# bentherien/point-cloud-reid

Hardware: AMD Instinct MI355X
Metric: siamese pair-comparisons/sec @1024 pts (higher is better)
Workload: dtype bf16x3

## Files before the change

point-cloud-reid_amd/csrc/attn_kernels_impl.h:

```cpp
#pragma once
#ifndef PCR_ATTN_PREC
#define PCR_ATTN_PREC 0
#endif
#include "tile_dense.h"

#include <stdio.h>

#include <vector>

namespace {
constexpr int kAPrec = PCR_ATTN_PREC;
struct AttnArgs {
  pcr_attn_params p;
  int dbg;
  int wpc;
};

constexpr int kATraceWgs = 512, kATraceRecs = 24, kATraceMarks = 8;
__device__ unsigned long long g_attn_trace[2 * kATraceWgs * kATraceRecs * kATraceMarks];


__device__ __forceinline__ void pos_hidden(float *dst, int RP, const float *P, const float *w0,
                                           const float *b0, int d, int T) {
  for (int e = threadIdx.x; e < d * T; e += blockDim.x) {
// ... 1346 lines not shown
          }
        }
    }
    __builtin_amdgcn_wave_barrier();
    PCR_AMARK(7);
    PCR_ANEXT();
  }
#undef PCR_AMARK
#undef PCR_ANEXT
}

template <int NB, bool TRANS = false>
__device__ __forceinline__ void ap128_step(f32x16 (&acc)[NB], const bf16x8 *wb, int ls, const bf16x8 &bh, const bf16x8 &bl) {
  auto mm = [](const bf16x8 &w, const bf16x8 &x, const f32x16 &c) __attribute__((always_inline)) {
    return TRANS ? __builtin_amdgcn_mfma_f32_32x32x16_bf16(x, w, c, 0, 0, 0) : __builtin_amdgcn_mfma_f32_32x32x16_bf16(w, x, c, 0, 0, 0);
  };
#pragma unroll
  for (int c0 = 0; c0 < NB; c0 += 4) {
    bf16x8 wh[4], wl[4];
#pragma unroll
    for (int cb = 0; cb < 4; cb++) {
      wh[cb] = wb[((ls * NB + c0 + cb) * 2) * 64];
      wl[cb] = wb[((ls * NB + c0 + cb) * 2 + 1) * 64];
    }
#pragma unroll
    for (int cb = 0; cb < 4; cb++) acc[c0 + cb] = mm(wh[cb], bh, acc[c0 + cb]);
#pragma unroll
    for (int cb = 0; cb < 4; cb++) acc[c0 + cb] = mm(wh[cb], bl, acc[c0 + cb]);
#pragma unroll
    for (int cb = 0; cb < 4; cb++) acc[c0 + cb] = mm(wl[cb], bh, acc[c0 + cb]);
    asm volatile("" ::: "memory");
  }
}
constexpr int kAp128Waves = 4, kAp128ChunkU = 2048, kAp128Chunks = 16;
constexpr int kAp128Npc = kAp128ChunkU / (64 * kAp128Waves);
__device__ __forceinline__ void ring128_fetch(f32x4 (&stg)[kAp128Npc], __amdgpu_buffer_rsrc_t r, int kk, int tid) {
#pragma unroll
  for (int u = 0; u < kAp128Npc; u++)
    stg[u] = __builtin_bit_cast(f32x4, __builtin_amdgcn_raw_buffer_load_b128(r, tid * 16, (kk * kAp128ChunkU + u * 64 * kAp128Waves) * 16, 0));
  asm volatile("" ::: "memory");
}
__device__ __forceinline__ void ring128_commit(f32x4 *s_ring, const f32x4 (&stg)[kAp128Npc], int k, int tid) {
  f32x4 *dst = s_ring + (k & 1) * kAp128ChunkU + tid;
#pragma unroll
  for (int u = 0; u < kAp128Npc; u++) dst[u * 64 * kAp128Waves] = stg[u];
  __syncthreads();
}
constexpr size_t kAp128Lds = (size_t)2 * kAp128ChunkU * 16 + (640 + 4 * 128 + kAp128Waves * 128) * sizeof(float);
template <int NH>
__global__ __launch_bounds__(64 * kAp128Waves) __attribute__((amdgpu_waves_per_eu(1, 1)))
void attn_apply_stream128_kernel(AttnArgs a) {
  constexpr int D = 128, ND = 4, SD = 8, GPH = 8 / NH;
  extern __shared__ __attribute__((aligned(16))) float smem[];
  const pcr_attn_params &p = a.p;
  f32x4 *s_ring = reinterpret_cast<f32x4 *>(smem);
  int coff = 2 * kAp128ChunkU * 4;
  asm volatile("" : "+s"(coff));
  float *s_c = smem + coff;
  f32x4 *s_p0 = reinterpret_cast<f32x4 *>(s_c + 640);
  float *s_ks = s_c + 640 + 4 * 128;
  const int tid = threadIdx.x, lane = tid & 63, j = lane & 31, h = lane >> 5;
  const int wave = __builtin_amdgcn_readfirstlane(tid >> 6);
  const __amdgpu_buffer_rsrc_t rwq = __builtin_amdgcn_make_buffer_rsrc(const_cast<float *>(p.wq), 0, 4 * kAp128ChunkU * 16, 0x00020000),
                               rw0 = __builtin_amdgcn_make_buffer_rsrc(const_cast<float *>(p.wmlp0), 0, 8 * kAp128ChunkU * 16, 0x00020000),
                               rw2 = __builtin_amdgcn_make_buffer_rsrc(const_cast<float *>(p.wmlp2), 0, 4 * kAp128ChunkU * 16, 0x00020000);
  f32x4 stg[kAp128Npc];
  auto fetch = [&](int k) __attribute__((always_inline)) {
    k %= kAp128Chunks;
    ring128_fetch(stg, k < 4 ? rwq : (k < 12 ? rw0 : rw2), k < 4 ? k : (k < 12 ? k - 4 : k - 12), tid);
  };
  auto commit = [&](int k) __attribute__((always_inline)) { ring128_commit(s_ring, stg, k, tid); };
  for (int e = tid; e < D; e += 64 * kAp128Waves) {
    s_c[e] = p.bq[e];
    s_c[128 + e] = p.ln1_g[e];
    s_c[256 + e] = p.ln1_b[e];
    s_c[384 + e] = p.ln2_g[e];
    s_c[512 + e] = p.ln2_b[e];
    s_p0[e] = f32x4{p.pos0_w[3 * e], p.pos0_w[3 * e + 1], p.pos0_w[3 * e + 2], p.pos0_b[e]};
  }
  fetch(0);
  commit(0);
  const int nblk = p.Lq >> 5;
  const long nitem = (long)p.B * nblk;
  const float skf = (float)p.Sk;
  float *ksw = s_ks + wave * 128;
  auto cvec = [&](const float *base, int cb, int g) __attribute__((always_inline)) {
    return *reinterpret_cast<const f32x4 *>(base + 32 * cb + 8 * g + 4 * h);
  };
  auto to_ops = [&](const f32x16 &acc, int G, bf16x8 &oh, bf16x8 &ol) __attribute__((always_inline)) {
    float v[8];
#pragma unroll
    for (int e = 0; e < 8; e++) v[e] = acc[8 * G + e];
    bf_split8(v, oh, ol, true);
  };
  auto layernorm = [&](f32x16 (&v)[ND], const float *gam, const float *bet) __attribute__((always_inline)) {
    float sm = 0.f;
#pragma unroll
    for (int cb = 0; cb < ND; cb++)
#pragma unroll
      for (int r = 0; r < 16; r++) sm += v[cb][r];
    sm += __shfl_xor(sm, 32, 64);
    const float mean = sm / (float)D;
    float vr = 0.f;
#pragma unroll
    for (int cb = 0; cb < ND; cb++)
#pragma unroll
      for (int r = 0; r < 16; r++) {
        const float dlt = v[cb][r] - mean;
        vr += dlt * dlt;
      }
    vr += __shfl_xor(vr, 32, 64);
    const float inv = 1.0f / sqrtf(vr / (float)D + 1e-5f);
#pragma unroll
    for (int cb = 0; cb < ND; cb++)
#pragma unroll
      for (int g = 0; g < 4; g++) {
        const f32x4 gv = cvec(gam, cb, g), bv = cvec(bet, cb, g);
#pragma unroll
        for (int qq = 0; qq < 4; qq++) v[cb][4 * g + qq] = (v[cb][4 * g + qq] - mean) * inv * gv[qq] + bv[qq];
      }
  };
  for (long it0 = (long)blockIdx.x * kAp128Waves; it0 < nitem; it0 += (long)gridDim.x * kAp128Waves) {
    const long item = it0 + wave;
    const bool live = item < nitem;
    const long it = live ? item : nitem - 1;
    const long b = it / nblk;
    const int blk = (int)(it - b * nblk);
    const size_t bq_ = p.q_index ? (size_t)p.q_index[b] : (size_t)b;
    const size_t kb_ = p.kv_index ? (size_t)p.kv_index[b] : (size_t)b;
    const float *kvp = p.kv + kb_ * ((size_t)D * D + D);
    const int t = blk * 32 + j;
    const __amdgpu_buffer_rsrc_t rfeat = __builtin_amdgcn_make_buffer_rsrc(
        const_cast<float *>(p.feat_q + bq_ * D * p.Lq), 0, D * p.Lq * 4, 0x00020000);
    const int vo = (4 * h * p.Lq + t) * 4;
    auto load_x = [&](float (&xf)[64]) __attribute__((always_inline)) {
#pragma unroll
      for (int e = 0; e < 64; e++) {
        const int ch = 16 * (e >> 3) + bf_kpos(0, e & 7);
        xf[e] = __builtin_bit_cast(float, __builtin_amdgcn_raw_buffer_load_b32(rfeat, vo, ch * p.Lq * 4, 0));
      }
    };
    ksw[lane] = kvp[(size_t)D * D + lane];
    ksw[64 + lane] = kvp[(size_t)D * D + 64 + lane];
    bf16x8 bh[16], bl[16];
    {
      float xf[64];
      load_x(xf);
      const float *xyz = p.xyz_q + (bq_ * p.Lq + t) * 3;
      const float px = xyz[0], py = xyz[1], pz = xyz[2];
#pragma unroll
      for (int s2 = 0; s2 < SD; s2++) {
        float hv[8];
#pragma unroll
        for (int e = 0; e < 8; e++) {
          const f32x4 w = s_p0[16 * s2 + bf_kpos(0, e) + 4 * h];
          const float v = w[0] * px + w[1] * py + w[2] * pz + w[3];
          hv[e] = relu_i(v);
        }
        bf_split8(hv, bh[SD + s2], bl[SD + s2], true);
      }
#pragma unroll
      for (int e = 0; e < 64; e++) asm volatile("" : "+v"(xf[e]));
#pragma unroll
      for (int s2 = 0; s2 < SD; s2++) {
        float xv[8];
#pragma unroll
        for (int e = 0; e < 8; e++) xv[e] = xf[8 * s2 + e];
        bf_split8(xv, bh[s2], bl[s2], true);
      }
    }
    f32x16 q[ND];
#pragma unroll
    for (int cb = 0; cb < ND; cb++)
#pragma unroll
      for (int g = 0; g < 4; g++) {
        const f32x4 bqv = cvec(s_c, cb, g);
#pragma unroll
        for (int qq = 0; qq < 4; qq++) q[cb][4 * g + qq] = bqv[qq];
      }
#pragma unroll
    for (int k = 0; k < 4; k++) {
      fetch(k + 1);
      const bf16x8 *wb = reinterpret_cast<const bf16x8 *>(s_ring + (k & 1) * kAp128ChunkU) + lane;
#pragma unroll
      for (int ls = 0; ls < 4; ls++) ap128_step<ND>(q, wb, ls, bh[4 * k + ls], bl[4 * k + ls]);
      commit(k + 1);
    }
    float zg[SD];
#pragma unroll
    for (int cb = 0; cb < ND; cb++)
#pragma unroll
      for (int g = 0; g < 4; g++) {
        const f32x4 ksv = cvec(ksw, cb, g);
        float zz = 0.f;
#pragma unroll
        for (int qq = 0; qq < 4; qq++) {
          const float v = elu1(q[cb][4 * g + qq]);
          q[cb][4 * g + qq] = v;
          zz += v * ksv[qq];
        }
        if ((g & 1) == 0) zg[2 * cb + (g >> 1)] = zz;
        else zg[2 * cb + (g >> 1)] += zz;
      }
    float zs[NH];
#pragma unroll
    for (int hd = 0; hd < NH; hd++) {
      float z = zg[hd * GPH];
#pragma unroll
      for (int gi = 1; gi < GPH; gi++) z += zg[hd * GPH + gi];
      z += __shfl_xor(z, 32, 64);
      zs[hd] = (1.0f / (z + 1e-6f)) * skf;
    }
#pragma unroll
    for (int cb = 0; cb < ND; cb++)
#pragma unroll
      for (int r = 0; r < 16; r++) q[cb][r] *= zs[(2 * cb + (r >> 3)) / GPH];
    {
      bf16x8 ch_[SD], cl_[SD];
#pragma unroll
      for (int cb = 0; cb < ND; cb++)
#pragma unroll
        for (int G = 0; G < 2; G++) to_ops(q[cb], G, ch_[2 * cb + G], cl_[2 * cb + G]);
#pragma unroll
      for (int cb = 0; cb < ND; cb++)
#pragma unroll
        for (int r = 0; r < 16; r++) q[cb][r] = 0.f;
      const bf16x8 *mb = reinterpret_cast<const bf16x8 *>(kvp) + lane;
      bf16x8 mh[2][ND], ml[2][ND];
#pragma unroll
      for (int cb = 0; cb < ND; cb++) {
        mh[0][cb] = mb[(cb * 2) * 64];
        ml[0][cb] = mb[(cb * 2 + 1) * 64];
      }
#pragma unroll
      for (int s2 = 0; s2 < SD; s2++) {
        const int c = s2 & 1;
        if (s2 + 1 < SD) {
#pragma unroll
          for (int cb = 0; cb < ND; cb++) {
            mh[c ^ 1][cb] = mb[(((s2 + 1) * ND + cb) * 2) * 64];
            ml[c ^ 1][cb] = mb[(((s2 + 1) * ND + cb) * 2 + 1) * 64];
          }
        }
        asm volatile("" ::: "memory");
#pragma unroll
        for (int cb = 0; cb < ND; cb++) q[cb] = __builtin_amdgcn_mfma_f32_32x32x16_bf16(mh[c][cb], ch_[s2], q[cb], 0, 0, 0);
#pragma unroll
        for (int cb = 0; cb < ND; cb++) q[cb] = __builtin_amdgcn_mfma_f32_32x32x16_bf16(mh[c][cb], cl_[s2], q[cb], 0, 0, 0);
#pragma unroll
        for (int cb = 0; cb < ND; cb++) q[cb] = __builtin_amdgcn_mfma_f32_32x32x16_bf16(ml[c][cb], ch_[s2], q[cb], 0, 0, 0);
      }
    }
    layernorm(q, s_c + 128, s_c + 256);
#pragma unroll
    for (int cb = 0; cb < ND; cb++)
#pragma unroll
      for (int G = 0; G < 2; G++) to_ops(q[cb], G, bh[SD + 2 * cb + G], bl[SD + 2 * cb + G]);
    f32x16 f[2 * ND];
#pragma unroll
    for (int cb = 0; cb < 2 * ND; cb++)
#pragma unroll
      for (int r = 0; r < 16; r++) f[cb][r] = 0.f;
#pragma unroll
    for (int k = 4; k < 12; k++) {
      fetch(k + 1);
      const bf16x8 *wb = reinterpret_cast<const bf16x8 *>(s_ring + (k & 1) * kAp128ChunkU) + lane;
#pragma unroll
      for (int ls = 0; ls < 2; ls++) ap128_step<2 * ND>(f, wb, ls, bh[2 * (k - 4) + ls], bl[2 * (k - 4) + ls]);
      commit(k + 1);
    }
    float xf[64];
    load_x(xf);
    f32x16 o[ND];
#pragma unroll
    for (int cb = 0; cb < ND; cb++)
#pragma unroll
      for (int r = 0; r < 16; r++) o[cb][r] = 0.f;
#pragma unroll
    for (int k = 12; k < 16; k++) {
      fetch(k + 1);
      bf16x8 oh[4], ol[4];
#pragma unroll
      for (int i = 0; i < 2; i++) {
        f32x16 &fc = f[2 * (k - 12) + i];
#pragma unroll
        for (int r = 0; r < 16; r++) fc[r] = relu_i(fc[r]);
#pragma unroll
        for (int G = 0; G < 2; G++) to_ops(fc, G, oh[2 * i + G], ol[2 * i + G]);
      }
      const bf16x8 *wb = reinterpret_cast<const bf16x8 *>(s_ring + (k & 1) * kAp128ChunkU) + lane;
#pragma unroll
      for (int ls = 0; ls < 4; ls++) ap128_step<ND>(o, wb, ls, oh[ls], ol[ls]);
      commit(k + 1);
    }
    layernorm(o, s_c + 384, s_c + 512);
#pragma unroll
    for (int cb = 0; cb < ND; cb++)
#pragma unroll
      for (int r = 0; r < 16; r++) o[cb][r] += xf[16 * cb + r];
    if (live) {
      const __amdgpu_buffer_rsrc_t rout =
          __builtin_amdgcn_make_buffer_rsrc(p.out + (size_t)b * D * p.Lq, 0, D * p.Lq * 4, 0x00020000);
#pragma unroll
      for (int e = 0; e < 16 * ND; e++) {
        const int ch = 16 * (e >> 3) + bf_kpos(0, e & 7);
        const float v = o[e >> 4][e & 15];
        __builtin_amdgcn_raw_buffer_store_b32(__builtin_bit_cast(unsigned, v), rout, vo, ch * p.Lq * 4, 0);
      }
    }
  }
}

__host__ __device__ constexpr int attn_kv128_wpc(int nblk) { return nblk >= 32 ? 4 : (nblk >= 16 ? 2 : 1); }
constexpr size_t kKv128Lds0 = (size_t)2 * kAp128ChunkU * 16 + 128 * 16 + 256 * 4;
template <int NH>
__global__ __launch_bounds__(64 * kAp128Waves) __attribute__((amdgpu_waves_per_eu(1, 1)))
void attn_kv_stream128_kernel(AttnArgs a) {
  constexpr int D = 128, SD = 8, TPH = 4 / NH, NKV = NH * TPH * TPH;
  constexpr int KVU = NKV * 16 + 4;
  typedef unsigned u32x4 __attribute__((ext_vector_type(4)));
  extern __shared__ __attribute__((aligned(16))) float smem[];
  const pcr_attn_params &p = a.p;
  f32x4 *s_ring = reinterpret_cast<f32x4 *>(smem);
  int coff = 2 * kAp128ChunkU * 4;
  asm volatile("" : "+s"(coff));
  f32x4 *s_p0 = reinterpret_cast<f32x4 *>(smem + coff);
  float *s_bkv = smem + coff + 4 * D;
  float *s_red = s_bkv + 2 * D;
  const int tid = threadIdx.x, lane = tid & 63, j = lane & 31, h = lane >> 5;
  const int wave = __builtin_amdgcn_readfirstlane(tid >> 6);
  const __amdgpu_buffer_rsrc_t rw = __builtin_amdgcn_make_buffer_rsrc(const_cast<float *>(p.wkv_bf), 0, 8 * kAp128ChunkU * 16, 0x00020000);
  f32x4 stg[kAp128Npc];
  auto fetch = [&](int k) __attribute__((always_inline)) { ring128_fetch(stg, rw, k & 7, tid); };
  auto commit = [&](int k) __attribute__((always_inline)) { ring128_commit(s_ring, stg, k, tid); };
  for (int e = tid; e < D; e += 64 * kAp128Waves) s_p0[e] = f32x4{p.pos0_w[3 * e], p.pos0_w[3 * e + 1], p.pos0_w[3 * e + 2], p.pos0_b[e]};
  for (int e = tid; e < 2 * D; e += 64 * kAp128Waves) s_bkv[e] = p.bkv[e];
  fetch(0);
  commit(0);
  const int Sk = p.Sk, nblk = Sk >> 5;
  const int wpc = a.wpc, cpg = kAp128Waves / wpc;
  const int cslot = wave / wpc, wsub = wave - cslot * wpc;
  const int nper = (nblk + wpc - 1) / wpc;
  const long cstep = (long)gridDim.x * cpg;
  const float inv_sk = 1.0f / (float)Sk;
  float xf[64], pxyz[3];
  auto issue = [&](long bq, int blk) __attribute__((always_inline)) {
    const __amdgpu_buffer_rsrc_t rfeat =
        __builtin_amdgcn_make_buffer_rsrc(const_cast<float *>(p.feat_k + (size_t)bq * D * Sk), 0, D * Sk * 4, 0x00020000);
    const int t = blk * 32 + j, vo = (4 * h * Sk + t) * 4;
#pragma unroll
    for (int e = 0; e < 64; e++) {
      const int ch = 16 * (e >> 3) + bf_kpos(0, e & 7);
      xf[e] = __builtin_bit_cast(float, __builtin_amdgcn_raw_buffer_load_b32(rfeat, vo, ch * Sk * 4, 0));
    }
    const __amdgpu_buffer_rsrc_t rxyz =
        __builtin_amdgcn_make_buffer_rsrc(const_cast<float *>(p.xyz_k + (size_t)bq * Sk * 3), 0, Sk * 12, 0x00020000);
#pragma unroll
    for (int c = 0; c < 3; c++) pxyz[c] = __builtin_bit_cast(float, __builtin_amdgcn_raw_buffer_load_b32(rxyz, t * 12, c * 4, 0));
    asm volatile("" ::: "memory");
  };
  if ((long)blockIdx.x * cpg + cslot < p.B && wsub < nblk) issue((long)blockIdx.x * cpg + cslot, wsub);
  for (long c0 = (long)blockIdx.x * cpg; c0 < p.B; c0 += cstep) {
    const long b = c0 + cslot;
    const bool live = b < p.B;
    f32x16 kv[NKV];
#pragma unroll
    for (int i = 0; i < NKV; i++)
#pragma unroll
      for (int r = 0; r < 16; r++) kv[i][r] = 0.f;
    float ks[4] = {0.f, 0.f, 0.f, 0.f};
    for (int it = 0; it < nper; it++) {
      const int blk = wsub + it * wpc;
      const bool has = live && blk < nblk;
      const bool last = it + 1 == nper;
      const long bn = last ? b + cstep : b;
      const int blkn = last ? wsub : blk + wpc;
      const bool hasn = bn < p.B && blkn < nblk;
      bf16x8 bh[SD], bl[SD];
      if (has) {
#pragma unroll
        for (int s2 = 0; s2 < SD; s2++) {
          float xv[8];
#pragma unroll
          for (int e = 0; e < 8; e++) xv[e] = xf[8 * s2 + e];
          bf_split8(xv, bh[s2], bl[s2], true);
        }
      }
      f32x16 acc[8];
#pragma unroll
      for (int cb = 0; cb < 8; cb++)
#pragma unroll
        for (int r = 0; r < 16; r++) acc[cb][r] = 0.f;
#pragma unroll
      for (int k = 0; k < 8; k++) {
        fetch(k + 1);
        if (has) {
          const bf16x8 *wb = reinterpret_cast<const bf16x8 *>(s_ring + (k & 1) * kAp128ChunkU) + lane;
#pragma unroll
          for (int ls = 0; ls < 2; ls++) {
            if (k < 4) {
              ap128_step<8, true>(acc, wb, ls, bh[2 * k + ls], bl[2 * k + ls]);
            } else {
              const int s2 = 2 * k + ls - SD;
              float hv[8];
#pragma unroll
              for (int e = 0; e < 8; e++) {
                const f32x4 w = s_p0[16 * s2 + bf_kpos(0, e) + 4 * h];
                const float v = w[0] * pxyz[0] + w[1] * pxyz[1] + w[2] * pxyz[2] + w[3];
                hv[e] = relu_i(v);
              }
              bf16x8 hh, hl;
              bf_split8(hv, hh, hl, true);
              ap128_step<8, true>(acc, wb, ls, hh, hl);
            }
          }
        }
        commit(k + 1);
      }
      if (hasn) issue(bn, blkn);
      else {
#pragma unroll
        for (int e = 0; e < 64; e++) xf[e] = 0.f;
        pxyz[0] = pxyz[1] = pxyz[2] = 0.f;
      }
      if (has) {
        float bias[8];
#pragma unroll
        for (int cb = 0; cb < 8; cb++) bias[cb] = s_bkv[cb * 32 + j];
#pragma unroll
        for (int r = 0; r < 16; r++) {
#pragma unroll
          for (int cb = 0; cb < 4; cb++) {
            acc[cb][r] = elu1(acc[cb][r] + bias[cb]);
            ks[cb] += acc[cb][r];
            acc[4 + cb][r] = (acc[4 + cb][r] + bias[4 + cb]) * inv_sk;
          }
        }
#pragma unroll
        for (int i = 0; i < NKV; i++) {
          const int hd = i / (TPH * TPH), ib = hd * TPH + (i % (TPH * TPH)) / TPH, jb = hd * TPH + i % TPH;
#pragma unroll
          for (int r = 0; r < 16; r++) kv[i] = __builtin_amdgcn_mfma_f32_32x32x2f32(acc[4 + jb][r], acc[ib][r], kv[i], 0, 0, 0);
        }
      }
    }
#pragma unroll
    for (int cb = 0; cb < 4; cb++) ks[cb] += __shfl_xor(ks[cb], 32, 64);
    if (wpc > 1) {
      int ln = lane;
      asm volatile("" : "+v"(ln));
      float *red = s_red + (size_t)cslot * KVU * 64 + ln;
      for (int round = 0; round < wpc; round++) {
        if (wsub == round) {
#pragma unroll
          for (int i = 0; i < NKV; i++)
#pragma unroll
            for (int r = 0; r < 16; r++) {
              float *dst = red + (i * 16 + r) * 64;
              *dst = round == 0 ? kv[i][r] : *dst + kv[i][r];
            }
#pragma unroll
          for (int cb = 0; cb < 4; cb++) {
            float *dst = red + (NKV * 16 + cb) * 64;
            *dst = round == 0 ? ks[cb] : *dst + ks[cb];
          }
        }
        __syncthreads();
      }
#pragma unroll
      for (int i = 0; i < NKV; i++)
#pragma unroll
        for (int r = 0; r < 16; r++) kv[i][r] = red[(i * 16 + r) * 64];
#pragma unroll
      for (int cb = 0; cb < 4; cb++) ks[cb] = red[(NKV * 16 + cb) * 64];
    }
    if (live) {
      int ln = lane;
      asm volatile("" : "+v"(ln));
      const int j = ln & 31, h = ln >> 5;
      const __amdgpu_buffer_rsrc_t rkv =
          __builtin_amdgcn_make_buffer_rsrc(p.kv + (size_t)b * ((size_t)D * D + D), 0, (D * D + D) * 4, 0x00020000);
      const __amdgpu_buffer_rsrc_t rwm = __builtin_amdgcn_make_buffer_rsrc(const_cast<float *>(p.wmerge), 0, D * D * 4, 0x00020000);
      for (int ob = wsub; ob < 4; ob += wpc) {
        const int wrow = ((ob * 32 + j) * D + 4 * h) * 4;
#pragma unroll
        for (int hd = 0; hd < NH; hd++) {
          f32x4 w[TPH][4];
#pragma unroll
          for (int jj = 0; jj < TPH; jj++)
#pragma unroll
            for (int g = 0; g < 4; g++)
              w[jj][g] = __builtin_bit_cast(f32x4, __builtin_amdgcn_raw_buffer_load_b128(rwm, wrow, ((hd * TPH + jj) * 32 + 8 * g) * 4, 0));
#pragma unroll
          for (int dl = 0; dl < TPH; dl++) {
            const int db = hd * TPH + dl;
            f32x16 m;
#pragma unroll
            for (int r = 0; r < 16; r++) m[r] = 0.f;
#pragma unroll
            for (int jj = 0; jj < TPH; jj++) {
              const int i = hd * TPH * TPH + dl * TPH + jj;
#pragma unroll
              for (int r = 0; r < 16; r++) m = __builtin_amdgcn_mfma_f32_32x32x2f32(kv[i][r], w[jj][r >> 2][r & 3], m, 0, 0, 0);
            }
#pragma unroll
            for (int G = 0; G < 2; G++) {
              float v[8];
#pragma unroll
              for (int e = 0; e < 8; e++) v[e] = m[8 * G + e];
              bf16x8 hi, lo;
              bf_split8(v, hi, lo, true);
              const int unit = (((db * 2 + G) * (D >> 5) + ob) * 2) * 64 + h * 32 + j;
              __builtin_amdgcn_raw_buffer_store_b128(__builtin_bit_cast(u32x4, hi), rkv, unit * 16, 0, 0);
              __builtin_amdgcn_raw_buffer_store_b128(__builtin_bit_cast(u32x4, lo), rkv, (unit + 64) * 16, 0, 0);
            }
          }
        }
      }
      if (wsub == 0 && h == 0) {
#pragma unroll
        for (int cb = 0; cb < 4; cb++)
          __builtin_amdgcn_raw_buffer_store_b32(__builtin_bit_cast(unsigned, ks[cb]), rkv, (D * D + cb * 32 + j) * 4, 0, 0);
      }
    }
  }
}
#endif

}

static int attn_check(const pcr_attn_params &p) {
  if (p.B < 0 || p.Lq < 1 || p.Sk < 1 || p.c1 < 1 || p.c2 < 1 || p.cout < 1 || p.nhead < 1) return 1;
  if (p.d < 32 || p.d > 512 || (p.d & 31) || p.d % p.nhead) return 1;
  if (p.d > 128 && ((p.d & 63) || ((p.d / p.nhead) & 63) || p.d / p.nhead > 256)) return 1;
  if ((p.c2 & 7) || p.cout > 512 || p.cfinal > 512) return 1;
  if (!p.feat_q || !p.feat_k || !p.xyz_k || !p.kv || !p.pos0_w || !p.pos0_b || !p.wq || !p.bq || !p.wkv ||
      !p.bkv || !p.wmerge || !p.wmlp0 || !p.wmlp2 || !p.ln1_g || !p.ln1_b || !p.ln2_g || !p.ln2_b)
    return 1;
  if (p.q_pos && (!p.xyz_q || p.c1 != p.c2 || p.c1 != p.d)) return 1;
  if (p.residual && p.cout != p.c1) return 1;
  if (p.cfinal && (!p.wfinal || !p.bfinal || (p.cout & 7))) return 1;
  return 0;
}

static void attn_dump_trace(const char *path, const char *tag, int wgs, int B, int Sk) {
  static int launches = 0;
  static const int skip = pcr_tune_int("PCR_SA_TRACE_SKIP");
  launches++;
  if (launches <= skip || launches > skip + 8) return;
  static std::vector<unsigned long long> host(2 * kATraceWgs * kATraceRecs * kATraceMarks);
  if (hipDeviceSynchronize() != hipSuccess) return;
  if (hipMemcpyFromSymbol(host.data(), HIP_SYMBOL(g_attn_trace), host.size() * sizeof(unsigned long long)) != hipSuccess) return;
  FILE *f = fopen(path, "a");
  if (!f) return;
  const int n = 2 * (wgs < kATraceWgs ? wgs : kATraceWgs);
  fprintf(f, "launch %d kernel %s wgs %d B %d Sk %d\n", launches, tag, wgs, B, Sk);
  for (int w = 0; w < n; w++) {
    const unsigned long long *t = host.data() + (size_t)w * (kATraceRecs * kATraceMarks);
// ... 60 lines not shown
    if (onew)
      rc = mh ? pcr_launch_lds<attn_kv_stream64_kernel<true, kBfUnit, 4, kBfUnit>>(gg, bb, lds_s, st, a)
              : pcr_launch_lds<attn_kv_stream64_kernel<false, kBfUnit, 4, kBfUnit>>(gg, bb, lds_s, st, a);
    else
      rc = mh ? pcr_launch_lds<attn_kv_stream64_kernel<true, kBfUnit>>(gg, bb, lds_s, st, a)
              : pcr_launch_lds<attn_kv_stream64_kernel<false, kBfUnit>>(gg, bb, lds_s, st, a);
    if (atrace) attn_dump_trace(atrace, "kv64", gs, (int)pp->B, pp->Sk);
    return rc;
  }
#if PCR_ATTN_PREC != 0
  if (ns == 1 && d == 32 && pp->c2 == 32 && pp->wkv_bf && (pp->Sk & 31) == 0 && pp->nhead >= 1 && 32 % pp->nhead == 0) {
    pcr_note_arith(PCR_PREC_BF16X3);
    const int nblk = pp->Sk >> 5;
    int wpc2 = 1;
    while (wpc2 * 2 <= (nblk < kKvsWaves ? nblk : kKvsWaves)) wpc2 *= 2;
    if (wpc2 < 2) wpc2 = 2;
    const int cpg = kKvsWaves / wpc2;
    const size_t lds_s = (size_t)(4096 + 128 + 64 + 32 * 33 + cpg * (32 * 33 + 32)) * sizeof(float);
    const long rounds = ((long)pp->B + cpg - 1) / cpg;
    const long cap = 2L * pcr_cu_count();
    return pcr_launch_lds<attn_kv_stream32_kernel>(dim3((unsigned)(rounds < cap ? rounds : cap)), dim3(64 * kKvsWaves), lds_s, st, a);
  }
  static const int no_kv128 = pcr_tune_int("PCR_ATTN_NO_KV128");
  if (ns == 1 && d == 128 && pp->c2 == 128 && pp->wkv_bf && (pp->Sk & 31) == 0 && pp->Sk >= 256 &&
      (pp->nhead == 2 || pp->nhead == 4) && !no_kv128) {
    pcr_note_arith(PCR_PREC_BF16X3);
    a.wpc = attn_kv128_wpc(pp->Sk >> 5);
    static const int wpc_t = pcr_tune_int("PCR_ATTN_KV128_WPC");
    if (wpc_t == 1 || wpc_t == 2 || wpc_t == 4) a.wpc = wpc_t;
    const int cpg = kAp128Waves / a.wpc;
    const size_t lds_s = kKv128Lds0 + (a.wpc > 1 ? (size_t)cpg * (16 * (16 / pp->nhead) + 4) * 64 * sizeof(float) : 0);
    const long nwg = ((long)pp->B + cpg - 1) / cpg;
    const dim3 gg((unsigned)(nwg < pcr_cu_count() ? nwg : pcr_cu_count())), bb(64 * kAp128Waves);
    return pp->nhead == 2 ? pcr_launch_lds<attn_kv_stream128_kernel<2>>(gg, bb, lds_s, st, a)
                          : pcr_launch_lds<attn_kv_stream128_kernel<4>>(gg, bb, lds_s, st, a);
  }
#endif
  pcr_note_arith(PCR_PREC_F32);
  int rc;
  if (d == 32) rc = pcr_launch_lds<attn_kv_kernel<2, 1, 2, 1>>(g, blk, lds, st, a);
  else if (d == 64) rc = pcr_launch_lds<attn_kv_kernel_o3<2, 1, 1, 1>>(g, blk, lds, st, a);
  else if (d == 128) {
    if (kBfUnit && pp->wkv_bf && pp->Sk >= 256) rc = pcr_launch_lds<attn_kv_kernel_o2<1, 2, 1, 4, true>>(g, blk, lds, st, a);
    else rc = pcr_launch_lds<attn_kv_kernel_o2<1, 2, 1, 4>>(g, blk, lds, st, a);
  }
  else rc = pcr_launch_lds<attn_kv_kernel<1, 2, 0, 4>>(g, blk, lds, st, a);
  if (rc != PCR_OK || ns == 1) return rc;
  return pcr_launch_lds<attn_kv_fold_kernel>(dim3(pp->B), blk, ((size_t)d * (d + 1) + d) * sizeof(float), st, a);
}

static bool aps64_shape(const pcr_attn_params &p) {
  const bool aps_in = p.c1 == 64 || ((p.c1 == 32 || (p.c1 < 16 && p.wmlp0_bf_xpad)) && !p.q_pos && !p.residual);
  const bool aps_out = (p.cout == 64 && (p.cfinal == 0 || p.cfinal == 128) && p.c1 >= 32) ||
                       (p.cout == 128 && !p.cfinal && !p.residual && p.c1 == 64) ||
                       (p.cout == 32 && p.cfinal == 64 && !p.residual && p.c1 < 16);
  return p.d == 64 && aps_in && aps_out && (p.Lq & 31) == 0 && (p.nhead == 1 || p.nhead == 2 || p.nhead == 4);
}

static int attn_apply_launch(const pcr_attn_params *pp, pcr_stream_t stream) {
  const pcr_attn_params &p = *pp;
  AttnArgs a;
  a.p = p;
  a.dbg = 0;
  a.wpc = 0;
  const int tb = p.d <= 32 ? 4 : (p.d <= 64 ? 2 : 1), T = 32 * tb, RP = T + 1;
  const int catP = ceil8(p.c1 + p.d);
  int rowsU = catP > 2 * p.d ? catP : 2 * p.d;
  if (ceil32(p.cout) > rowsU) rowsU = ceil32(p.cout);
  if (ceil32(p.cfinal) > rowsU) rowsU = ceil32(p.cfinal);
  size_t lds = ((size_t)(rowsU + 3 + p.nhead) * RP + 2 * (kThreads / T) * T + 7 * p.d + 2 * p.cout) *
               sizeof(float);
  if (lds > (size_t)kMaxDynLds) return PCR_ERR_INVALID;
  dim3 g((p.Lq + T - 1) / T, p.B), blk(kThreads);
  hipStream_t st = pcr_s(stream);
  pcr_note_arith(kAPrec != 0 ? PCR_PREC_BF16X3 : PCR_PREC_F32);
#if PCR_ATTN_PREC != 0
  const int aps_c1s = (p.c1 + 15) >> 4, aps_nd = p.d >> 5;
  const size_t aps_lds = (size_t)((aps_c1s + (p.q_pos ? 2 * aps_nd : 0)) * aps_nd * 128 + (aps_c1s + 2 * aps_nd) * aps_nd * 256 +
                                  aps_nd * (p.cout >> 5) * 512) * 16 +
                         (size_t)(448 + 256 + 64 * kApsWaves) * sizeof(float);
  static const int no_s128 = pcr_tune_int("PCR_ATTN_NO_STREAM128");
  if (p.d == 128 && p.c1 == 128 && p.cout == 128 && !p.cfinal && p.q_pos && p.residual && (p.Lq & 31) == 0 && p.Lq >= 256 &&
      (p.nhead == 1 || p.nhead == 2 || p.nhead == 4) && !no_s128) {
    const long nitem = (long)p.B * (p.Lq >> 5);
    const long nwg = (nitem + kAp128Waves - 1) / kAp128Waves;
    const dim3 gg((unsigned)(nwg < pcr_cu_count() ? nwg : pcr_cu_count())), bb(64 * kAp128Waves);
    if (p.nhead == 1) return pcr_launch_lds<attn_apply_stream128_kernel<1>>(gg, bb, kAp128Lds, st, a);
    if (p.nhead == 2) return pcr_launch_lds<attn_apply_stream128_kernel<2>>(gg, bb, kAp128Lds, st, a);
    return pcr_launch_lds<attn_apply_stream128_kernel<4>>(gg, bb, kAp128Lds, st, a);
  }
  if (p.d == 32 && p.c1 == 32 && p.cout == 32 && !p.cfinal && (p.Lq & 31) == 0 && (p.nhead == 1 || p.nhead == 2)) {
    const long nitem = (long)p.B * (p.Lq >> 5);
    const long nwg = (nitem + kApsWaves - 1) / kApsWaves;
    const dim3 gg((unsigned)(nwg < pcr_cu_count() ? nwg : pcr_cu_count())), bb(64 * kApsWaves);
    return p.q_pos ? pcr_launch_lds<attn_apply_stream64_kernel<true, 2, 0, 1, 1>>(gg, bb, aps_lds, st, a)
                   : pcr_launch_lds<attn_apply_stream64_kernel<false, 2, 0, 1, 1>>(gg, bb, aps_lds, st, a);
  }
  if (aps64_shape(p) && aps_lds <= (size_t)kMaxDynLds) {
    const int nob = p.cout >> 5;
    const long nitem = (long)p.B * (p.Lq >> 5);
    const long nwg = (nitem + kApsWaves - 1) / kApsWaves;
    const dim3 gg((unsigned)(nwg < pcr_cu_count() ? nwg : pcr_cu_count())), bb(64 * kApsWaves);
    const bool cf = p.cfinal != 0;
    static const char *aptrace = pcr_tune_str("PCR_ATTN_TRACE");
    if (aptrace) a.dbg = 256;
    if (pp->pool_out) {
      const long nwgp = ((long)p.B + kApsWaves - 1) / kApsWaves;
      const dim3 ggp((unsigned)(nwgp < pcr_cu_count() ? nwgp : pcr_cu_count()));
      return pcr_launch_lds<attn_apply_stream64_kernel<false, 4, 0, 2, 2, true>>(ggp, bb, aps_lds, st, a);
    }
    int rc;
    if (nob == 4)
      rc = p.q_pos ? pcr_launch_lds<attn_apply_stream64_kernel<true, 4, 0, 4>>(gg, bb, aps_lds, st, a)
                   : pcr_launch_lds<attn_apply_stream64_kernel<false, 4, 0, 4>>(gg, bb, aps_lds, st, a);
    else if (p.c1 < 16) rc = pcr_launch_lds<attn_apply_stream64_kernel<false, 1, 2, 1>>(gg, bb, aps_lds, st, a);
    else if (p.c1 == 32)
      rc = cf ? pcr_launch_lds<attn_apply_stream64_kernel<false, 2, 4>>(gg, bb, aps_lds, st, a)
              : pcr_launch_lds<attn_apply_stream64_kernel<false, 2, 0>>(gg, bb, aps_lds, st, a);
    else if (p.q_pos)
// ... 95 lines not shown
```

Before: 66300.

## Pipeline d128 attention kernels with direct-to-LDS weight ring and prefetching

Reworks the d=128 attention apply and kv stream kernels to overlap memory with MFMA work. Weight chunks now go straight from global memory into the LDS ring via buffer-load-to-LDS, removing the register staging and copy. A software-pipelined chunk routine keeps the next weight fragments in registers and uses sched_barrier to interleave the loads with the MFMAs. Next-item features, coordinates and kv scale are prefetched a full iteration ahead, kv matrix loads go one step deeper, and the merge weights are double-buffered. Old paths stay selectable through a tuning flag. The cost is more register pressure and more complex sync ordering.

```diff
diff --git a/point-cloud-reid_amd/csrc/attn_kernels_impl.h b/point-cloud-reid_amd/csrc/attn_kernels_impl.h
--- a/point-cloud-reid_amd/csrc/attn_kernels_impl.h
+++ b/point-cloud-reid_amd/csrc/attn_kernels_impl.h
@@ -1402,6 +1402,81 @@
     asm volatile("" ::: "memory");
   }
 }
+constexpr int kD128OldOps = 1, kD128OldFold = 2, kD128OldAhead = 4, kD128OldRing = 8;
+struct Ap128W {
+  bf16x8 h[4], l[4];
+};
+__device__ __forceinline__ void ap128_prime(Ap128W &w, const bf16x8 *wb) {
+#pragma unroll
+  for (int cb = 0; cb < 4; cb++) {
+    w.h[cb] = wb[(2 * cb) * 64];
+    w.l[cb] = wb[(2 * cb + 1) * 64];
+  }
+}
+template <int NB, int NLS, bool TRANS, bool OLD, class OPS, class EDGE>
+__device__ __forceinline__ void ap128_chunk(f32x16 (&acc)[NB], Ap128W &w, const bf16x8 *wb, const bf16x8 *wbn, OPS ops, EDGE edge,
+                                            bool carry = true) {
+  if (OLD) {
+#pragma unroll
+    for (int ls = 0; ls < NLS; ls++) {
+      bf16x8 xh, xl;
+      ops(ls, xh, xl);
+      ap128_step<NB, TRANS>(acc, wb, ls, xh, xl);
+    }
+    edge();
+    return;
+  }
+  constexpr int GPS = NB / 4, NG = NLS * GPS;
+  constexpr int kPin = 0x2 | 0x4 | 0x10 | 0x400;
+  auto mm = [](const bf16x8 &w, const bf16x8 &x, const f32x16 &c) __attribute__((always_inline)) {
+    return TRANS ? __builtin_amdgcn_mfma_f32_32x32x16_bf16(x, w, c, 0, 0, 0) : __builtin_amdgcn_mfma_f32_32x32x16_bf16(w, x, c, 0, 0, 0);
+  };
+  bf16x8 (&wh)[4] = w.h, (&wl)[4] = w.l;
+  bf16x8 xh, xl, nxh, nxl;
+  ops(0, nxh, nxl);
+#pragma unroll
+  for (int g = 0; g < NG; g++) {
+    const int c0 = (g % GPS) * 4;
+    const bool more = g + 1 < NG;
+    const bf16x8 *wn = more ? wb + 8 * (g + 1) * 64 : wbn;
+    if (g % GPS == 0) {
+      xh = nxh;
+      xl = nxl;
+    }
+    if (g % GPS == GPS - 1 && more) ops(g / GPS + 1, nxh, nxl);
+    __builtin_amdgcn_sched_barrier(kPin);
+#pragma unroll
+    for (int c2 = 0; c2 < 4; c2 += 2) {
+#pragma unroll
+      for (int cb = c2; cb < c2 + 2; cb++) acc[c0 + cb] = mm(wh[cb], xh, acc[c0 + cb]);
+      __builtin_amdgcn_sched_barrier(kPin);
+      if (!more && c2 == 0) {
+#pragma unroll
+        for (int cb = 0; cb < 2; cb++) acc[c0 + cb] = mm(wh[cb], xl, acc[c0 + cb]);
+        __builtin_amdgcn_sched_barrier(0);
+        edge();
+        __builtin_amdgcn_sched_barrier(0);
+#pragma unroll
+        for (int cb = 0; cb < 2; cb++)
+          if (carry) wh[cb] = wn[(2 * cb) * 64];
+        __builtin_amdgcn_sched_barrier(kPin);
+        continue;
+      }
+#pragma unroll
+      for (int cb = c2; cb < c2 + 2; cb++) {
+        acc[c0 + cb] = mm(wh[cb], xl, acc[c0 + cb]);
+        if (more || carry) wh[cb] = wn[(2 * cb) * 64];
+        __builtin_amdgcn_sched_barrier(kPin);
+      }
+    }
+#pragma unroll
+    for (int cb = 0; cb < 4; cb++) {
+      acc[c0 + cb] = mm(wl[cb], xh, acc[c0 + cb]);
+      if (more || carry) wl[cb] = wn[(2 * cb + 1) * 64];
+      __builtin_amdgcn_sched_barrier(kPin);
+    }
+  }
+}
 constexpr int kAp128Waves = 4, kAp128ChunkU = 2048, kAp128Chunks = 16;
 constexpr int kAp128Npc = kAp128ChunkU / (64 * kAp128Waves);
 __device__ __forceinline__ void ring128_fetch(f32x4 (&stg)[kAp128Npc], __amdgpu_buffer_rsrc_t r, int kk, int tid) {
@@ -1416,11 +1491,19 @@
   for (int u = 0; u < kAp128Npc; u++) dst[u * 64 * kAp128Waves] = stg[u];
   __syncthreads();
 }
+__device__ __forceinline__ void ring128_fetch_lds(f32x4 *s_ring, __amdgpu_buffer_rsrc_t r, int kk, int k, int tid, int wave) {
+#pragma unroll
+  for (int u = 0; u < kAp128Npc; u++)
+    __builtin_amdgcn_raw_ptr_buffer_load_lds(
+        r, (__attribute__((address_space(3))) void *)(s_ring + (k & 1) * kAp128ChunkU + (u * kAp128Waves + wave) * 64), 16, tid * 16,
+        (kk * kAp128ChunkU + u * 64 * kAp128Waves) * 16, 0, 0);
+}
 constexpr size_t kAp128Lds = (size_t)2 * kAp128ChunkU * 16 + (640 + 4 * 128 + kAp128Waves * 128) * sizeof(float);
-template <int NH>
+template <int NH, int OLD = 0>
 __global__ __launch_bounds__(64 * kAp128Waves) __attribute__((amdgpu_waves_per_eu(1, 1)))
 void attn_apply_stream128_kernel(AttnArgs a) {
   constexpr int D = 128, ND = 4, SD = 8, GPH = 8 / NH;
+  constexpr bool kOldOps = (OLD & kD128OldOps) != 0, kOldAhead = (OLD & kD128OldAhead) != 0, kOldRing = (OLD & kD128OldRing) != 0;
   extern __shared__ __attribute__((aligned(16))) float smem[];
   const pcr_attn_params &p = a.p;
   f32x4 *s_ring = reinterpret_cast<f32x4 *>(smem);
@@ -1437,9 +1520,14 @@
   f32x4 stg[kAp128Npc];
   auto fetch = [&](int k) __attribute__((always_inline)) {
     k %= kAp128Chunks;
-    ring128_fetch(stg, k < 4 ? rwq : (k < 12 ? rw0 : rw2), k < 4 ? k : (k < 12 ? k - 4 : k - 12), tid);
+    const int kk = k < 4 ? k : (k < 12 ? k - 4 : k - 12);
+    if (kOldRing) ring128_fetch(stg, k < 4 ? rwq : (k < 12 ? rw0 : rw2), kk, tid);
+    else ring128_fetch_lds(s_ring, k < 4 ? rwq : (k < 12 ? rw0 : rw2), kk, k, tid, wave);
   };
-  auto commit = [&](int k) __attribute__((always_inline)) { ring128_commit(s_ring, stg, k, tid); };
+  auto commit = [&](int k) __attribute__((always_inline)) {
+    if (kOldRing) ring128_commit(s_ring, stg, k, tid);
+    else __syncthreads();
+  };
   for (int e = tid; e < D; e += 64 * kAp128Waves) {
     s_c[e] = p.bq[e];
     s_c[128 + e] = p.ln1_g[e];
@@ -1450,6 +1538,10 @@
   }
   fetch(0);
   commit(0);
+  fetch(1);
+  auto slot = [&](int k) __attribute__((always_inline)) { return reinterpret_cast<const bf16x8 *>(s_ring + (k & 1) * kAp128ChunkU) + lane; };
+  Ap128W wreg;
+  if (!kOldOps) ap128_prime(wreg, slot(0));
   const int nblk = p.Lq >> 5;
   const long nitem = (long)p.B * nblk;
   const float skf = (float)p.Sk;
@@ -1490,34 +1582,59 @@
         for (int qq = 0; qq < 4; qq++) v[cb][4 * g + qq] = (v[cb][4 * g + qq] - mean) * inv * gv[qq] + bv[qq];
       }
   };
-  for (long it0 = (long)blockIdx.x * kAp128Waves; it0 < nitem; it0 += (long)gridDim.x * kAp128Waves) {
+  struct Item {
+    long b;
+    int t, vo;
+    __amdgpu_buffer_rsrc_t rfeat;
+    const float *xyz, *kvp;
+  };
+  auto locate = [&](long it0) __attribute__((always_inline)) {
     const long item = it0 + wave;
-    const bool live = item < nitem;
-    const long it = live ? item : nitem - 1;
-    const long b = it / nblk;
-    const int blk = (int)(it - b * nblk);
-    const size_t bq_ = p.q_index ? (size_t)p.q_index[b] : (size_t)b;
-    const size_t kb_ = p.kv_index ? (size_t)p.kv_index[b] : (size_t)b;
-    const float *kvp = p.kv + kb_ * ((size_t)D * D + D);
-    const int t = blk * 32 + j;
-    const __amdgpu_buffer_rsrc_t rfeat = __builtin_amdgcn_make_buffer_rsrc(
-        const_cast<float *>(p.feat_q + bq_ * D * p.Lq), 0, D * p.Lq * 4, 0x00020000);
-    const int vo = (4 * h * p.Lq + t) * 4;
-    auto load_x = [&](float (&xf)[64]) __attribute__((always_inline)) {
-#pragma unroll
-      for (int e = 0; e < 64; e++) {
-        const int ch = 16 * (e >> 3) + bf_kpos(0, e & 7);
-        xf[e] = __builtin_bit_cast(float, __builtin_amdgcn_raw_buffer_load_b32(rfeat, vo, ch * p.Lq * 4, 0));
-      }
-    };
-    ksw[lane] = kvp[(size_t)D * D + lane];
-    ksw[64 + lane] = kvp[(size_t)D * D + 64 + lane];
+    const long it = item < nitem ? item : nitem - 1;
+    Item w;
+    w.b = it / nblk;
+    const int blk = (int)(it - w.b * nblk);
+    const size_t bq_ = p.q_index ? (size_t)p.q_index[w.b] : (size_t)w.b;
+    const size_t kb_ = p.kv_index ? (size_t)p.kv_index[w.b] : (size_t)w.b;
+    w.kvp = p.kv + kb_ * ((size_t)D * D + D);
+    w.t = blk * 32 + j;
+    w.rfeat = __builtin_amdgcn_make_buffer_rsrc(const_cast<float *>(p.feat_q + bq_ * D * p.Lq), 0, D * p.Lq * 4, 0x00020000);
+    w.vo = (4 * h * p.Lq + w.t) * 4;
+    w.xyz = p.xyz_q + (bq_ * p.Lq + w.t) * 3;
+    return w;
+  };
+  auto load_x = [&](const Item &w, float (&xf)[64]) __attribute__((always_inline)) {
+#pragma unroll
+    for (int e = 0; e < 64; e++) {
+      const int ch = 16 * (e >> 3) + bf_kpos(0, e & 7);
+      xf[e] = __builtin_bit_cast(float, __builtin_amdgcn_raw_buffer_load_b32(w.rfeat, w.vo, ch * p.Lq * 4, 0));
+    }
+  };
+  float xnext[64], pnext[3], knext[2];
+  auto request = [&](long it0) __attribute__((always_inline)) {
+    const Item w = locate(it0);
+    load_x(w, xnext);
+#pragma unroll
+    for (int c = 0; c < 3; c++) pnext[c] = w.xyz[c];
+    knext[0] = w.kvp[(size_t)D * D + lane];
+    knext[1] = w.kvp[(size_t)D * D + 64 + lane];
+    asm volatile("" ::: "memory");
+  };
+  const long itstep = (long)gridDim.x * kAp128Waves;
+  if (!kOldAhead) request((long)blockIdx.x * kAp128Waves);
+  for (long it0 = (long)blockIdx.x * kAp128Waves; it0 < nitem; it0 += itstep) {
+    const bool live = it0 + wave < nitem;
+    const Item cur = locate(it0);
+    const long b = cur.b;
+    const float *kvp = cur.kvp;
+    const int vo = cur.vo;
+    if (kOldAhead) request(it0);
+    ksw[lane] = knext[0];
+    ksw[64 + lane] = knext[1];
     bf16x8 bh[16], bl[16];
     {
-      float xf[64];
-      load_x(xf);
-      const float *xyz = p.xyz_q + (bq_ * p.Lq + t) * 3;
-      const float px = xyz[0], py = xyz[1], pz = xyz[2];
+      float (&xf)[64] = xnext;
+      const float px = pnext[0], py = pnext[1], pz = pnext[2];
 #pragma unroll
       for (int s2 = 0; s2 < SD; s2++) {
         float hv[8];
@@ -1550,11 +1667,28 @@
       }
 #pragma unroll
     for (int k = 0; k < 4; k++) {
-      fetch(k + 1);
-      const bf16x8 *wb = reinterpret_cast<const bf16x8 *>(s_ring + (k & 1) * kAp128ChunkU) + lane;
-#pragma unroll
-      for (int ls = 0; ls < 4; ls++) ap128_step<ND>(q, wb, ls, bh[4 * k + ls], bl[4 * k + ls]);
-      commit(k + 1);
+      ap128_chunk<ND, 4, false, kOldOps>(q, wreg, slot(k), slot(k + 1), [&](int ls, bf16x8 &xh, bf16x8 &xl) __attribute__((always_inline)) {
+        xh = bh[4 * k + ls];
+        xl = bl[4 * k + ls];
+      }, [&]() __attribute__((always_inline)) {
+        commit(k + 1);
+        fetch(k + 2);
+      });
+    }
+    constexpr int MD = kOldAhead ? 1 : 2;
+    const bf16x8 *mb = reinterpret_cast<const bf16x8 *>(kvp) + lane;
+    bf16x8 mh[MD + 1][ND], ml[MD + 1][ND];
+    auto load_m = [&](int s2) __attribute__((always_inline)) {
+#pragma unroll
+      for (int cb = 0; cb < ND; cb++) {
+        mh[s2 % (MD + 1)][cb] = mb[((s2 * ND + cb) * 2) * 64];
+        ml[s2 % (MD + 1)][cb] = mb[((s2 * ND + cb) * 2 + 1) * 64];
+      }
+    };
+    if (!kOldAhead) {
+#pragma unroll
+      for (int s2 = 0; s2 < MD; s2++) load_m(s2);
+      asm volatile("" ::: "memory");
     }
     float zg[SD];
 #pragma unroll
@@ -1595,23 +1729,11 @@
       for (int cb = 0; cb < ND; cb++)
 #pragma unroll
         for (int r = 0; r < 16; r++) q[cb][r] = 0.f;
-      const bf16x8 *mb = reinterpret_cast<const bf16x8 *>(kvp) + lane;
-      bf16x8 mh[2][ND], ml[2][ND];
-#pragma unroll
-      for (int cb = 0; cb < ND; cb++) {
-        mh[0][cb] = mb[(cb * 2) * 64];
-        ml[0][cb] = mb[(cb * 2 + 1) * 64];
-      }
+      if (kOldAhead) load_m(0);
 #pragma unroll
       for (int s2 = 0; s2 < SD; s2++) {
-        const int c = s2 & 1;
-        if (s2 + 1 < SD) {
-#pragma unroll
-          for (int cb = 0; cb < ND; cb++) {
-            mh[c ^ 1][cb] = mb[(((s2 + 1) * ND + cb) * 2) * 64];
-            ml[c ^ 1][cb] = mb[(((s2 + 1) * ND + cb) * 2 + 1) * 64];
-          }
-        }
+        const int c = s2 % (MD + 1);
+        if (s2 + MD < SD) load_m(s2 + MD);
         asm volatile("" ::: "memory");
 #pragma unroll
         for (int cb = 0; cb < ND; cb++) q[cb] = __builtin_amdgcn_mfma_f32_32x32x16_bf16(mh[c][cb], ch_[s2], q[cb], 0, 0, 0);
@@ -1633,14 +1755,16 @@
       for (int r = 0; r < 16; r++) f[cb][r] = 0.f;
 #pragma unroll
     for (int k = 4; k < 12; k++) {
-      fetch(k + 1);
-      const bf16x8 *wb = reinterpret_cast<const bf16x8 *>(s_ring + (k & 1) * kAp128ChunkU) + lane;
-#pragma unroll
-      for (int ls = 0; ls < 2; ls++) ap128_step<2 * ND>(f, wb, ls, bh[2 * (k - 4) + ls], bl[2 * (k - 4) + ls]);
-      commit(k + 1);
+      ap128_chunk<2 * ND, 2, false, kOldOps>(f, wreg, slot(k), slot(k + 1), [&](int ls, bf16x8 &xh, bf16x8 &xl) __attribute__((always_inline)) {
+        xh = bh[2 * (k - 4) + ls];
+        xl = bl[2 * (k - 4) + ls];
+      }, [&]() __attribute__((always_inline)) {
+        commit(k + 1);
+        fetch(k + 2);
+      });
     }
     float xf[64];
-    load_x(xf);
+    load_x(cur, xf);
     f32x16 o[ND];
 #pragma unroll
     for (int cb = 0; cb < ND; cb++)
@@ -1648,7 +1772,6 @@
       for (int r = 0; r < 16; r++) o[cb][r] = 0.f;
 #pragma unroll
     for (int k = 12; k < 16; k++) {
-      fetch(k + 1);
       bf16x8 oh[4], ol[4];
 #pragma unroll
       for (int i = 0; i < 2; i++) {
@@ -1658,11 +1781,15 @@
 #pragma unroll
         for (int G = 0; G < 2; G++) to_ops(fc, G, oh[2 * i + G], ol[2 * i + G]);
       }
-      const bf16x8 *wb = reinterpret_cast<const bf16x8 *>(s_ring + (k & 1) * kAp128ChunkU) + lane;
-#pragma unroll
-      for (int ls = 0; ls < 4; ls++) ap128_step<ND>(o, wb, ls, oh[ls], ol[ls]);
-      commit(k + 1);
-    }
+      ap128_chunk<ND, 4, false, kOldOps>(o, wreg, slot(k), slot(k + 1), [&](int ls, bf16x8 &xh, bf16x8 &xl) __attribute__((always_inline)) {
+        xh = oh[ls];
+        xl = ol[ls];
+      }, [&]() __attribute__((always_inline)) {
+        commit(k + 1);
+        fetch(k + 2);
+      });
+    }
+    if (!kOldAhead) request(it0 + itstep);
     layernorm(o, s_c + 384, s_c + 512);
 #pragma unroll
     for (int cb = 0; cb < ND; cb++)
@@ -1679,14 +1806,16 @@
       }
     }
   }
+  asm volatile("s_waitcnt vmcnt(0)" ::: "memory");
 }
 
 __host__ __device__ constexpr int attn_kv128_wpc(int nblk) { return nblk >= 32 ? 4 : (nblk >= 16 ? 2 : 1); }
 constexpr size_t kKv128Lds0 = (size_t)2 * kAp128ChunkU * 16 + 128 * 16 + 256 * 4;
-template <int NH>
+template <int NH, int OLD = 0>
 __global__ __launch_bounds__(64 * kAp128Waves) __attribute__((amdgpu_waves_per_eu(1, 1)))
 void attn_kv_stream128_kernel(AttnArgs a) {
   constexpr int D = 128, SD = 8, TPH = 4 / NH, NKV = NH * TPH * TPH;
+  constexpr bool kOldOps = (OLD & kD128OldOps) != 0, kOldFold = (OLD & kD128OldFold) != 0, kOldRing = (OLD & kD128OldRing) != 0;
   constexpr int KVU = NKV * 16 + 4;
   typedef unsigned u32x4 __attribute__((ext_vector_type(4)));
   extern __shared__ __attribute__((aligned(16))) float smem[];
@@ -1701,12 +1830,20 @@
   const int wave = __builtin_amdgcn_readfirstlane(tid >> 6);
   const __amdgpu_buffer_rsrc_t rw = __builtin_amdgcn_make_buffer_rsrc(const_cast<float *>(p.wkv_bf), 0, 8 * kAp128ChunkU * 16, 0x00020000);
   f32x4 stg[kAp128Npc];
-  auto fetch = [&](int k) __attribute__((always_inline)) { ring128_fetch(stg, rw, k & 7, tid); };
-  auto commit = [&](int k) __attribute__((always_inline)) { ring128_commit(s_ring, stg, k, tid); };
+  auto fetch = [&](int k) __attribute__((always_inline)) {
+    if (kOldRing) ring128_fetch(stg, rw, k & 7, tid);
+    else ring128_fetch_lds(s_ring, rw, k & 7, k, tid, wave);
+  };
+  auto commit = [&](int k) __attribute__((always_inline)) {
+    if (kOldRing) ring128_commit(s_ring, stg, k, tid);
+    else __syncthreads();
+  };
   for (int e = tid; e < D; e += 64 * kAp128Waves) s_p0[e] = f32x4{p.pos0_w[3 * e], p.pos0_w[3 * e + 1], p.pos0_w[3 * e + 2], p.pos0_b[e]};
   for (int e = tid; e < 2 * D; e += 64 * kAp128Waves) s_bkv[e] = p.bkv[e];
   fetch(0);
   commit(0);
+  fetch(1);
+  auto slot = [&](int k) __attribute__((always_inline)) { return reinterpret_cast<const bf16x8 *>(s_ring + (k & 1) * kAp128ChunkU) + lane; };
   const int Sk = p.Sk, nblk = Sk >> 5;
   const int wpc = a.wpc, cpg = kAp128Waves / wpc;
   const int cslot = wave / wpc, wsub = wave - cslot * wpc;
@@ -1746,30 +1883,26 @@
       const long bn = last ? b + cstep : b;
       const int blkn = last ? wsub : blk + wpc;
       const bool hasn = bn < p.B && blkn < nblk;
-      bf16x8 bh[SD], bl[SD];
-      if (has) {
-#pragma unroll
-        for (int s2 = 0; s2 < SD; s2++) {
-          float xv[8];
-#pragma unroll
-          for (int e = 0; e < 8; e++) xv[e] = xf[8 * s2 + e];
-          bf_split8(xv, bh[s2], bl[s2], true);
-        }
-      }
       f32x16 acc[8];
+      Ap128W wreg;
 #pragma unroll
       for (int cb = 0; cb < 8; cb++)
 #pragma unroll
         for (int r = 0; r < 16; r++) acc[cb][r] = 0.f;
 #pragma unroll
       for (int k = 0; k < 8; k++) {
-        fetch(k + 1);
+        auto edge = [&]() __attribute__((always_inline)) {
+          commit(k + 1);
+          fetch(k + 2);
+        };
         if (has) {
-          const bf16x8 *wb = reinterpret_cast<const bf16x8 *>(s_ring + (k & 1) * kAp128ChunkU) + lane;
-#pragma unroll
-          for (int ls = 0; ls < 2; ls++) {
+          if (!kOldOps && k == 0) ap128_prime(wreg, slot(0));
+          ap128_chunk<8, 2, true, kOldOps>(acc, wreg, slot(k), slot(k + 1), [&](int ls, bf16x8 &xh, bf16x8 &xl) __attribute__((always_inline)) {
             if (k < 4) {
-              ap128_step<8, true>(acc, wb, ls, bh[2 * k + ls], bl[2 * k + ls]);
+              float xv[8];
+#pragma unroll
+              for (int e = 0; e < 8; e++) xv[e] = xf[8 * (2 * k + ls) + e];
+              bf_split8(xv, xh, xl, true);
             } else {
               const int s2 = 2 * k + ls - SD;
               float hv[8];
@@ -1779,13 +1912,12 @@
                 const float v = w[0] * pxyz[0] + w[1] * pxyz[1] + w[2] * pxyz[2] + w[3];
                 hv[e] = relu_i(v);
               }
-              bf16x8 hh, hl;
-              bf_split8(hv, hh, hl, true);
-              ap128_step<8, true>(acc, wb, ls, hh, hl);
+              bf_split8(hv, xh, xl, true);
             }
-          }
-        }
-        commit(k + 1);
+          }, edge, k < 7);
+        } else {
+          edge();
+        }
       }
       if (hasn) issue(bn, blkn);
       else {
@@ -1851,16 +1983,24 @@
       const __amdgpu_buffer_rsrc_t rkv =
           __builtin_amdgcn_make_buffer_rsrc(p.kv + (size_t)b * ((size_t)D * D + D), 0, (D * D + D) * 4, 0x00020000);
       const __amdgpu_buffer_rsrc_t rwm = __builtin_amdgcn_make_buffer_rsrc(const_cast<float *>(p.wmerge), 0, D * D * 4, 0x00020000);
+      auto load_w = [&](f32x4 (&w)[TPH][4], int ob, int hd) __attribute__((always_inline)) {
+        const int wrow = ((ob * 32 + j) * D + 4 * h) * 4;
+#pragma unroll
+        for (int jj = 0; jj < TPH; jj++)
+#pragma unroll
+          for (int g = 0; g < 4; g++)
+            w[jj][g] = __builtin_bit_cast(f32x4, __builtin_amdgcn_raw_buffer_load_b128(rwm, wrow, ((hd * TPH + jj) * 32 + 8 * g) * 4, 0));
+      };
+      f32x4 w[TPH][4], wn[TPH][4];
+      if (!kOldFold) load_w(w, wsub, 0);
       for (int ob = wsub; ob < 4; ob += wpc) {
-        const int wrow = ((ob * 32 + j) * D + 4 * h) * 4;
 #pragma unroll
         for (int hd = 0; hd < NH; hd++) {
-          f32x4 w[TPH][4];
-#pragma unroll
-          for (int jj = 0; jj < TPH; jj++)
-#pragma unroll
-            for (int g = 0; g < 4; g++)
-              w[jj][g] = __builtin_bit_cast(f32x4, __builtin_amdgcn_raw_buffer_load_b128(rwm, wrow, ((hd * TPH + jj) * 32 + 8 * g) * 4, 0));
+          if (kOldFold) load_w(w, ob, hd);
+          else {
+            load_w(wn, hd + 1 < NH ? ob : (ob + wpc < 4 ? ob + wpc : ob), (hd + 1) % NH);
+            asm volatile("" ::: "memory");
+          }
 #pragma unroll
           for (int dl = 0; dl < TPH; dl++) {
             const int db = hd * TPH + dl;
@@ -1885,6 +2025,12 @@
               __builtin_amdgcn_raw_buffer_store_b128(__builtin_bit_cast(u32x4, lo), rkv, (unit + 64) * 16, 0, 0);
             }
           }
+          if (!kOldFold) {
+#pragma unroll
+            for (int jj = 0; jj < TPH; jj++)
+#pragma unroll
+              for (int g = 0; g < 4; g++) w[jj][g] = wn[jj][g];
+          }
         }
       }
       if (wsub == 0 && h == 0) {
@@ -1894,6 +2040,7 @@
       }
     }
   }
+  asm volatile("s_waitcnt vmcnt(0)" ::: "memory");
 }
 #endif
 
@@ -2020,6 +2167,14 @@
     const size_t lds_s = kKv128Lds0 + (a.wpc > 1 ? (size_t)cpg * (16 * (16 / pp->nhead) + 4) * 64 * sizeof(float) : 0);
     const long nwg = ((long)pp->B + cpg - 1) / cpg;
     const dim3 gg((unsigned)(nwg < pcr_cu_count() ? nwg : pcr_cu_count())), bb(64 * kAp128Waves);
+#if PCR_TUNING
+    static const int old128 = pcr_tune_int("PCR_ATTN_D128_OLD");
+    constexpr int kAll = kD128OldOps | kD128OldFold | kD128OldRing;
+    if (pp->nhead == 2 && (old128 & kAll) == kD128OldOps) return pcr_launch_lds<attn_kv_stream128_kernel<2, kD128OldOps>>(gg, bb, lds_s, st, a);
+    if (pp->nhead == 2 && (old128 & kAll) == kD128OldFold) return pcr_launch_lds<attn_kv_stream128_kernel<2, kD128OldFold>>(gg, bb, lds_s, st, a);
+    if (pp->nhead == 2 && (old128 & kAll) == kD128OldRing) return pcr_launch_lds<attn_kv_stream128_kernel<2, kD128OldRing>>(gg, bb, lds_s, st, a);
+    if (pp->nhead == 2 && (old128 & kAll) == kAll) return pcr_launch_lds<attn_kv_stream128_kernel<2, kAll>>(gg, bb, lds_s, st, a);
+#endif
     return pp->nhead == 2 ? pcr_launch_lds<attn_kv_stream128_kernel<2>>(gg, bb, lds_s, st, a)
                           : pcr_launch_lds<attn_kv_stream128_kernel<4>>(gg, bb, lds_s, st, a);
   }
@@ -2073,6 +2228,14 @@
     const long nitem = (long)p.B * (p.Lq >> 5);
     const long nwg = (nitem + kAp128Waves - 1) / kAp128Waves;
     const dim3 gg((unsigned)(nwg < pcr_cu_count() ? nwg : pcr_cu_count())), bb(64 * kAp128Waves);
+#if PCR_TUNING
+    static const int old128 = pcr_tune_int("PCR_ATTN_D128_OLD");
+    constexpr int kAll = kD128OldOps | kD128OldAhead | kD128OldRing;
+    if (p.nhead == 2 && (old128 & kAll) == kD128OldOps) return pcr_launch_lds<attn_apply_stream128_kernel<2, kD128OldOps>>(gg, bb, kAp128Lds, st, a);
+    if (p.nhead == 2 && (old128 & kAll) == kD128OldAhead) return pcr_launch_lds<attn_apply_stream128_kernel<2, kD128OldAhead>>(gg, bb, kAp128Lds, st, a);
+    if (p.nhead == 2 && (old128 & kAll) == kD128OldRing) return pcr_launch_lds<attn_apply_stream128_kernel<2, kD128OldRing>>(gg, bb, kAp128Lds, st, a);
+    if (p.nhead == 2 && (old128 & kAll) == kAll) return pcr_launch_lds<attn_apply_stream128_kernel<2, kAll>>(gg, bb, kAp128Lds, st, a);
+#endif
     if (p.nhead == 1) return pcr_launch_lds<attn_apply_stream128_kernel<1>>(gg, bb, kAp128Lds, st, a);
     if (p.nhead == 2) return pcr_launch_lds<attn_apply_stream128_kernel<2>>(gg, bb, kAp128Lds, st, a);
     return pcr_launch_lds<attn_apply_stream128_kernel<4>>(gg, bb, kAp128Lds, st, a);
```

Result: no change. 66850 (median of 6 runs) (+0.8%).
